# Aedelon/ProteinBERT-PyTorch-Replication

Measured on AMD Instinct MI355X. Metric: sequences/sec (whole node) ProteinBERT pretrain L=512 at 1/2/4/8 MI355X, higher is better.
Workload: dtype bf16; 1 GPU; global_batch=2048, per_gpu_batch=2048, seq_len=512, parallelism=dp1, impl=hip, hip_graph=False

## Files before the change

### proteinbert_pytorch_replication_amd/ops/csrc/wgrad.hip

```cpp
#include "mfma.h"
#include <stdlib.h>

using namespace pbx;
typedef unsigned short bf16_t;

namespace {
constexpr int CH = 128;

constexpr int BM = 128;
constexpr int KS = 9;

__device__ __attribute__((aligned(16))) unsigned int g_zero16[4];
__device__ __attribute__((aligned(16))) unsigned int g_ones16[4] = {~0u, ~0u, ~0u, ~0u};

__device__ __forceinline__ void glds16(const void* src, unsigned char* lds_base) {
  const unsigned dst = __builtin_amdgcn_readfirstlane(
      (unsigned)(size_t)(__attribute__((address_space(3))) unsigned char*)lds_base);
  unsigned keep;
  asm volatile("s_mov_b32 %0, m0\n\ts_mov_b32 m0, %2\n\ts_nop 0\n\tglobal_load_lds_dwordx4 %1, off\n\ts_mov_b32 m0, %0"
               : "=&s"(keep)
               : "v"(src), "s"(dst)
               : "memory");
}

template <int NTAP, int BIAS, typename StageF>
__device__ __forceinline__ void wgrad_tiles(unsigned char* smem, int buf_bytes, long t0, long t1, StageF& stage,
                                            f32x16_t (&acc0)[5], f32x16_t (&acc1)[5], float& bsum, int halo,
                                            int d, int k0, int cig, int lane) {
  const int h = lane >> 5, q = tr_q(lane), tc = tr_c(lane);
  const int aoff = (8 * h + q) * 64 + tc * 2;
  int xoff[NTAP], xoff4[NTAP];
#pragma unroll
  for (int j = 0; j < NTAP; ++j) {
    const int rb = halo + 8 * h + q + (k0 + j - KS / 2) * d;
    xoff[j] = BM * 128 + swz256e(rb, cig * 32 + tc);
    xoff4[j] = BM * 128 + swz256e(rb + 4, cig * 32 + tc);
  }
  if (t0 < t1) stage(t0, smem);
  for (long tile = t0; tile < t1; ++tile) {
    unsigned char* cur = smem + ((tile - t0) & 1) * buf_bytes;
    unsigned char* nxt = smem + (((tile - t0) & 1) ^ 1) * buf_bytes;
    asm volatile("s_waitcnt vmcnt(0)" ::: "memory");
    __syncthreads();
    if (tile + 1 < t1) stage(tile + 1, nxt);
    constexpr int NS = (BM / 16) * NTAP;
    bf16x8 fa0[2], fa1[2], fb[3];
    auto read_a = [&](int kk) {
      const unsigned char* c = cur + kk * 16 * 64;
      fa0[kk & 1] = cat_tr(lds_tr(c, aoff), lds_tr(c, aoff + 256));
      fa1[kk & 1] = cat_tr(lds_tr(c, BM * 64 + aoff), lds_tr(c, BM * 64 + aoff + 256));
    };
    auto read_b = [&](int st) {
      const unsigned char* cx = cur + (st / NTAP) * 16 * 256;
      fb[st % 3] = cat_tr(lds_tr(cx, xoff[st % NTAP]), lds_tr(cx, xoff4[st % NTAP]));
    };
    read_a(0);
    read_b(0);
    read_b(1);
#pragma unroll
    for (int st = 0; st < NS; ++st) {
      const int kk = st / NTAP, j = st % NTAP;
      if (st + 2 < NS) {
        if ((st + 2) % NTAP == 0) read_a((st + 2) / NTAP);
        read_b(st + 2);
      }
      __builtin_amdgcn_sched_barrier(0);
      if (BIAS != 0 && j == 0) {
        typedef __attribute__((ext_vector_type(4))) unsigned int u32x4;
        const u32x4 u = __builtin_bit_cast(u32x4, BIAS == 2 ? fa1[kk & 1] : fa0[kk & 1]);
#pragma unroll
        for (int e = 0; e < 4; ++e)
          bsum += __builtin_bit_cast(float, u[e] << 16) + __builtin_bit_cast(float, u[e] & 0xffff0000u);
      }
      acc0[j] = mfma32(fa0[kk & 1], fb[st % 3], acc0[j]);
      acc1[j] = mfma32(fa1[kk & 1], fb[st % 3], acc1[j]);
    }
  }
}

__global__ void __launch_bounds__(512, 1) wgrad2_kernel(const bf16_t* __restrict__ dy0, const bf16_t* __restrict__ dy1,
                                                        const bf16_t* __restrict__ x, float* __restrict__ slab,
                                                        float* __restrict__ bslab, int B, int L, int dil1,
                                                        int nconv, int R, int buf_bytes, int xlo, int xhi) {
  extern __shared__ __attribute__((aligned(16))) unsigned char smem[];
  const int ntypes = nconv * 2;
  int type, chunk;
  if ((R & 7) == 0) {
    const int id = blockIdx.x, j = id >> 3;
    chunk = (j / ntypes) * 8 + (id & 7);
    type = j - (j / ntypes) * ntypes;
  } else {
    chunk = blockIdx.x / ntypes;
    type = blockIdx.x - chunk * ntypes;
  }
  const int cv = type >> 1, half = type & 1;
  const bf16_t* dy = cv ? dy1 : dy0;
  const int d = cv ? dil1 : 1;
  const int halo = (KS / 2) * d;
  const int XR = BM + 2 * halo;
  const int tid = threadIdx.x, lane = tid & 63, w = __builtin_amdgcn_readfirstlane(tid >> 6);
  const int r = lane & 31, h = lane >> 5;
  const int cig = w & 3;
  const int k0 = w < 4 ? 0 : 5;
  const int ntap = w < 4 ? 5 : 4;
  const int T = (L + BM - 1) / BM;
  const long NT = (long)B * T;
  const long t0 = NT * chunk / R, t1 = NT * (chunk + 1) / R;

  auto stage = [&](long tile, unsigned char* buf) {
    const int b = (int)(tile / T), t = (int)(tile - (tile / T) * T);
    const int pos0 = t * BM;
    const size_t sbase = (size_t)b * L * CH;
    const int n = 16 + XR / 4;
    for (int i = w; i < n; i += 8) {
      if (i < 16) {
        const int sub = i >> 3, row = (i & 7) * 16 + (lane >> 2);
        const int pos = pos0 + row;
        const void* src = pos < L ? (const void*)(dy + sbase + (size_t)pos * CH + half * 64 + sub * 32 + (lane & 3) * 8)
                                  : (const void*)g_zero16;
        glds16(src, buf + sub * (BM * 64) + (i & 7) * 1024);
      } else {
        const int j = i - 16, row = j * 4 + (lane >> 4);
        const int chunk16 = (lane & 15) ^ (((row & 3) << 2) | ((row >> 2) & 3));
        const int pos = pos0 - halo + row;
        const void* src = (pos >= -xlo && pos < L + xhi)
                              ? (const void*)(x + ((ptrdiff_t)b * (L + xlo + xhi) + xlo + pos) * CH + chunk16 * 8)
                              : (const void*)g_zero16;
        glds16(src, buf + BM * 128 + j * 1024);
      }
    }
  };

  f32x16_t acc0[5], acc1[5];
#pragma unroll
  for (int j = 0; j < 5; ++j) {
    acc0[j] = zero16();
    acc1[j] = zero16();
  }
  float bsum = 0.f;
  if (w == 0)
    wgrad_tiles<5, 1>(smem, buf_bytes, t0, t1, stage, acc0, acc1, bsum, halo, d, 0, cig, lane);
  else if (w == 1)
    wgrad_tiles<5, 2>(smem, buf_bytes, t0, t1, stage, acc0, acc1, bsum, halo, d, 0, cig, lane);
  else if (w < 4)
    wgrad_tiles<5, 0>(smem, buf_bytes, t0, t1, stage, acc0, acc1, bsum, halo, d, 0, cig, lane);
  else
    wgrad_tiles<4, 0>(smem, buf_bytes, t0, t1, stage, acc0, acc1, bsum, halo, d, 5, cig, lane);
  float* dst = slab + ((size_t)chunk * nconv + cv) * KS * CH * CH + cig * 32 + r;
#pragma unroll
  for (int j = 0; j < 5; ++j) {
    if (j < ntap) {
      const int k = k0 + j;
#pragma unroll
      for (int i = 0; i < 16; ++i) {
        const int co = half * 64 + (i & 3) + 8 * (i >> 2) + 4 * h;
        dst[((size_t)k * CH + co) * CH] = acc0[j][i];
        dst[((size_t)k * CH + co + 32) * CH] = acc1[j][i];
      }
    }
  }
  if (w < 2) {
    bsum += __shfl_xor(bsum, 32, 64);
    if (h == 0) bslab[((size_t)chunk * nconv + cv) * CH + half * 64 + w * 32 + r] = bsum;
  }
}

__global__ void __launch_bounds__(256) wgrad2_reduce_kernel(const float4* __restrict__ slab,
                                                            const float* __restrict__ bslab, float* __restrict__ dw0,
                                                            float* __restrict__ dw1, float* __restrict__ db0,
                                                            float* __restrict__ db1, int R, int nconv) {
  constexpr int per4 = KS * CH * CH / 4;
  const int total4 = nconv * per4;
  const int nblk_w = (total4 + 63) / 64;
  const int tid = threadIdx.x, col = tid & 63, part = tid >> 6;
  if ((int)blockIdx.x >= nblk_w) {
    const int idx = ((int)blockIdx.x - nblk_w) * 256 + tid;
    if (idx < nconv * CH) {
      float s = 0.f;
      for (int rr = 0; rr < R; ++rr) s += bslab[(size_t)rr * nconv * CH + idx];
      float* db = idx >= CH ? db1 : db0;
      if (db != nullptr) db[idx % CH] += s;
    }
    return;
  }
  __shared__ float4 red[4][64];
  const int idx = blockIdx.x * 64 + col;
  const int r0 = R * part / 4, r1 = R * (part + 1) / 4;
  float4 s = make_float4(0.f, 0.f, 0.f, 0.f);
  if (idx < total4) {
    int rr = r0;
    for (; rr + 8 <= r1; rr += 8) {
      float4 v[8];
#pragma unroll
      for (int u = 0; u < 8; ++u) v[u] = slab[(size_t)(rr + u) * total4 + idx];
#pragma unroll
      for (int u = 0; u < 8; ++u) {
        s.x += v[u].x; s.y += v[u].y; s.z += v[u].z; s.w += v[u].w;
      }
    }
    for (; rr < r1; ++rr) {
      const float4 a = slab[(size_t)rr * total4 + idx];
      s.x += a.x; s.y += a.y; s.z += a.z; s.w += a.w;
    }
  }
  red[part][col] = s;
  __syncthreads();
  if (part == 0 && idx < total4) {
#pragma unroll
    for (int p = 1; p < 4; ++p) {
      const float4 a = red[p][col];
      s.x += a.x; s.y += a.y; s.z += a.z; s.w += a.w;
    }
    const int cv = idx >= per4;
    const int rem = idx - cv * per4;
    const int k = rem / (CH * CH / 4), co = (rem / (CH / 4)) % CH, ci = (rem % (CH / 4)) * 4;
    float* dw = (cv ? dw1 : dw0) + ((size_t)co * CH + ci) * KS + k;
    dw[0] += s.x;
    dw[KS] += s.y;
    dw[2 * KS] += s.z;
    dw[3 * KS] += s.w;
  }
}

bool wgrad2_attr_set = false;
}

PBX_EXPORT int pbx_wgrad2x(const void* dy0, const void* dy1, const void* x, float* slab, float* bslab, float* dw0,
                           float* dw1, float* db0, float* db1, int B, int L, int dil1, int nconv, int R, int xlo,
                           int xhi, hipStream_t st) {
  if (nconv < 1 || nconv > 2 || R < 1 || dil1 < 1 || xlo < 0 || xhi < 0) return (int)hipErrorInvalidValue;
  const int halo_max = (KS / 2) * (nconv > 1 ? dil1 : 1);
  const int buf = BM * 128 + (BM + 2 * halo_max) * 256;
  if (2 * buf > 163840) return (int)hipErrorInvalidValue;
  if (!wgrad2_attr_set) {
    (void)hipFuncSetAttribute((const void*)wgrad2_kernel, hipFuncAttributeMaxDynamicSharedMemorySize, 163840);
    wgrad2_attr_set = true;
  }
  hipLaunchKernelGGL(wgrad2_kernel, dim3(nconv * 2 * R), dim3(512), 2 * buf, st, (const bf16_t*)dy0,
                     (const bf16_t*)dy1, (const bf16_t*)x, slab, bslab, B, L, dil1, nconv, R, buf, xlo, xhi);
  const int total4 = nconv * KS * CH * CH / 4;
  const int nblk = (total4 + 63) / 64 + (nconv * CH + 255) / 256;
  hipLaunchKernelGGL(wgrad2_reduce_kernel, dim3(nblk), dim3(256), 0, st, (const float4*)slab,
                     bslab, dw0, dw1, db0, db1, R, nconv);
  return pbx_launch_status();
}

PBX_EXPORT int pbx_wgrad2(const void* dy0, const void* dy1, const void* x, float* slab, float* bslab, float* dw0,
                          float* dw1, float* db0, float* db1, int B, int L, int dil1, int nconv, int R,
                          hipStream_t st) {
  return pbx_wgrad2x(dy0, dy1, x, slab, bslab, dw0, dw1, db0, db1, B, L, dil1, nconv, R, 0, 0, st);
}

namespace {
constexpr int TBM = 128;

__global__ void __launch_bounds__(512, 1) wgrad_tok_kernel(const long long* __restrict__ tok,
                                                           const bf16_t* __restrict__ dy0,
                                                           const bf16_t* __restrict__ dy1, float* __restrict__ slab,
                                                           int B, int L, int dil1, int R, int V, int buf_bytes) {
  extern __shared__ __attribute__((aligned(16))) unsigned char smem[];
  const int tid = threadIdx.x, lane = tid & 63, w = __builtin_amdgcn_readfirstlane(tid >> 6);
  const int r = lane & 31, h = lane >> 5;
  const int q = tr_q(lane), tc = tr_c(lane);
  const int cv = w >> 2, ct = w & 3;
  const int d = cv ? dil1 : 1;
  const int hal0 = KS / 2, hal1 = (KS / 2) * dil1;
  const int rows0 = TBM + 2 * hal0, rows1 = TBM + 2 * hal1;
  const int T = (L + TBM - 1) / TBM;
  const long NT = (long)B * T;
  const long t0 = NT * blockIdx.x / R, t1 = NT * (blockIdx.x + 1) / R;

  auto stage = [&](long tile, unsigned char* buf) {
    const int b = (int)(tile / T), t = (int)(tile - (tile / T) * T);
    const int pos0 = t * TBM;
    const size_t sbase = (size_t)b * L * CH;
    const int n0 = rows0 / 4, n1 = rows1 / 4;
    for (int i = w; i <= n0 + n1; i += 8) {
      if (i == n0 + n1) {
        const int p = pos0 + 2 * lane;
        const void* src = p < L ? (const void*)(tok + (size_t)b * L + p) : (const void*)g_ones16;
        glds16(src, buf + (rows0 + rows1) * 256);
        continue;
      }
      const int c = i >= n0;
      const int j = c ? i - n0 : i;
      const int hal = c ? hal1 : hal0;
      const bf16_t* dy = c ? dy1 : dy0;
      const int row = j * 4 + (lane >> 4);
      const int chunk16 = (lane & 15) ^ (((row & 3) << 2) | ((row >> 2) & 3));
      const int pos = pos0 - hal + row;
      const void* src = (pos >= 0 && pos < L) ? (const void*)(dy + sbase + (size_t)pos * CH + chunk16 * 8)
                                              : (const void*)g_zero16;
      glds16(src, buf + (c ? rows0 * 256 : 0) + j * 1024);
    }
  };

  f32x16_t acc[KS];
#pragma unroll
  for (int k = 0; k < KS; ++k) acc[k] = zero16();
  const int hal = cv ? hal1 : hal0;
  const int colb = ct * 32 + tc;
  const int cvb = cv ? rows0 * 256 : 0;
  int boff[KS], boff4[KS];
#pragma unroll
  for (int k = 0; k < KS; ++k) {
    const int rb = hal + (KS / 2 - k) * d + 8 * h + q;
    boff[k] = cvb + swz256e(rb, colb);
    boff4[k] = cvb + swz256e(rb + 4, colb);
  }
  const int toff = (rows0 + rows1) * 256 + 8 * h * 8;
  if (t0 < t1) stage(t0, smem);
  for (long tile = t0; tile < t1; ++tile) {
    unsigned char* cur = smem + ((tile - t0) & 1) * buf_bytes;
    unsigned char* nxt = smem + (((tile - t0) & 1) ^ 1) * buf_bytes;
    asm volatile("s_waitcnt vmcnt(0)" ::: "memory");
    __syncthreads();
    if (tile + 1 < t1) stage(tile + 1, nxt);
    constexpr int NS = (TBM / 16) * KS;
    bf16x8 fb[3], fa[2];
    unsigned tk[8];
    auto read_b = [&](int st) {
      const unsigned char* c = cur + (st / KS) * 4096;
      fb[st % 3] = cat_tr(lds_tr(c, boff[st % KS]), lds_tr(c, boff4[st % KS]));
    };
    auto read_tok = [&](int kb) {
      const unsigned* tp = reinterpret_cast<const unsigned*>(cur + toff + kb * 128);
#pragma unroll
      for (int j = 0; j < 8; ++j) tk[j] = tp[2 * j];
    };
    auto make_a = [&](int kb) {
      typedef __attribute__((ext_vector_type(4))) unsigned int u32x4;
      u32x4 o;
#pragma unroll
      for (int e = 0; e < 4; ++e)
        o[e] = (tk[2 * e] == (unsigned)r ? 0x3F80u : 0u) | (tk[2 * e + 1] == (unsigned)r ? 0x3F800000u : 0u);
      fa[kb & 1] = __builtin_bit_cast(bf16x8, o);
    };
    read_tok(0);
    make_a(0);
    read_b(0);
    read_b(1);
#pragma unroll
    for (int st = 0; st < NS; ++st) {
      const int kb = st / KS, k = st % KS;
      if (st + 2 < NS) read_b(st + 2);
      if (k == 3 && kb + 1 < TBM / 16) read_tok(kb + 1);
      if (k == 7 && kb + 1 < TBM / 16) make_a(kb + 1);
      __builtin_amdgcn_sched_barrier(0);
      acc[k] = mfma32(fa[kb & 1], fb[st % 3], acc[k]);
    }
  }
#pragma unroll
  for (int k = 0; k < KS; ++k)
#pragma unroll
    for (int i = 0; i < 16; ++i) {
      const int v = (i & 3) + 8 * (i >> 2) + 4 * h;
      if (v < V) slab[((((size_t)blockIdx.x * 2 + cv) * KS + k) * V + v) * CH + ct * 32 + r] = acc[k][i];
    }
}

__global__ void __launch_bounds__(128) wgrad_tok_finish_kernel(const float* __restrict__ S, const float* __restrict__ E,
                                                               float* __restrict__ dw0, float* __restrict__ dw1,
                                                               float* __restrict__ db0, float* __restrict__ db1,
                                                               int V, const float* __restrict__ W0,
                                                               const float* __restrict__ W1, float* __restrict__ dEslab) {
  __shared__ float sv[KS * 32];
  const int c = blockIdx.x / CH, co = blockIdx.x % CH, ci = threadIdx.x;
  for (int i = threadIdx.x; i < KS * V; i += 128) {
    const int k = i / V, v = i % V;
    sv[k * 32 + v] = S[(((size_t)c * KS + k) * V + v) * CH + co];
  }
  __syncthreads();
  float o[KS];
#pragma unroll
  for (int k = 0; k < KS; ++k) o[k] = 0.f;
  for (int v = 0; v < V; ++v) {
    const float e = bfround(E[v * CH + ci]);
#pragma unroll
    for (int k = 0; k < KS; ++k) o[k] = fmaf(e, sv[k * 32 + v], o[k]);
  }
  float* dw = (c ? dw1 : dw0) + ((size_t)co * CH + ci) * KS;
#pragma unroll
  for (int k = 0; k < KS; ++k) dw[k] += o[k];
  if (ci == 0) {
    float s = 0.f;
    for (int v = 0; v < V; ++v) s += sv[(KS / 2) * 32 + v];
    (c ? db1 : db0)[co] += s;
  }
  if (dEslab != nullptr) {
    const float* wr = (c ? W1 : W0) + ((size_t)co * CH + ci) * KS;
    float wk[KS];
#pragma unroll
    for (int k = 0; k < KS; ++k) wk[k] = bfround(wr[k]);
    for (int v = 0; v < V; ++v) {
      float a = 0.f;
#pragma unroll
      for (int k = 0; k < KS; ++k) a = fmaf(wk[k], sv[k * 32 + v], a);
      dEslab[((size_t)blockIdx.x * V + v) * CH + ci] = a;
    }
  }
}

bool wgrad_tok_attr_set = false;
}

extern "C" int pbx_colsum_add(const float* src, int rows, int cols, float* dst, const float* scale, hipStream_t st);
extern "C" int pbx_colsum_set(const float* src, int rows, int cols, float* dst, const float* scale, hipStream_t st);

PBX_EXPORT int pbx_wgrad_tok_rows(int B, int L) {
  constexpr int cap = 256;
  const long NT = (long)B * ((L + TBM - 1) / TBM);
  return (int)(NT < cap ? NT : cap);
}

PBX_EXPORT int pbx_wgrad_tok(const void* tok, const void* dy0, const void* dy1, const float* E, float* slab, float* S,
                             float* dw0, float* dw1, float* db0, float* db1, int B, int L, int dil1, int V,
                             const float* W0, const float* W1, float* dE, float* dEslab, hipStream_t st) {
  if (V < 1 || V > 32 || dil1 < 1 || (L & 1) || B < 1 || L < 1) return (int)hipErrorInvalidValue;
  if ((dE == nullptr) != (W0 == nullptr) || (dE == nullptr) != (W1 == nullptr) || (dE == nullptr) != (dEslab == nullptr))
    return (int)hipErrorInvalidValue;
  const int buf = (2 * TBM + 8 + 8 * dil1) * 256 + 1024;
  if (2 * buf > 163840) return (int)hipErrorInvalidValue;
  if (!wgrad_tok_attr_set) {
    (void)hipFuncSetAttribute((const void*)wgrad_tok_kernel, hipFuncAttributeMaxDynamicSharedMemorySize, 163840);
    wgrad_tok_attr_set = true;
  }
  const int R = pbx_wgrad_tok_rows(B, L);
  hipLaunchKernelGGL(wgrad_tok_kernel, dim3(R), dim3(512), 2 * buf, st, (const long long*)tok, (const bf16_t*)dy0,
                     (const bf16_t*)dy1, slab, B, L, dil1, R, V, buf);
  const int cols = 2 * KS * V * CH;
  int rc = pbx_colsum_set(slab, R, cols, S, nullptr, st);
  if (rc != 0) return rc;
  hipLaunchKernelGGL(wgrad_tok_finish_kernel, dim3(2 * CH), dim3(128), 0, st, S, E, dw0, dw1, db0, db1, V, W0, W1,
                     dEslab);
  if (dE == nullptr) return pbx_launch_status();
  rc = pbx_launch_status();
  if (rc != 0) return rc;
  return pbx_colsum_add(dEslab, 2 * CH, V * CH, dE, nullptr, st);
}
```

### proteinbert_pytorch_replication_amd/ops/local_track.py

```python
from __future__ import annotations

import ctypes
import os
from typing import List, Dict, Optional, Tuple

import torch

from . import _lib, streams
from ..train.arena import notify_grads_ready
from ..utils.determinism import fused_deterministic
from .global_track import bf16_of

_P, _I, _F, _L = ctypes.c_void_p, ctypes.c_int, ctypes.c_float, ctypes.c_long

_lib.register("pbx_conv_fwd3x", [_P, _P, _P, _P, _P, _P, _P, _P, _P, _P, _I, _I, _I, _I, _I, _I, _P])
_lib.register("pbx_conv_fwd5x", [_P, _P, _P, _P, _P, _P, _P, _P, _P, _P, _I, _I, _I, _I, _I, _I, _P])
_lib.register("pbx_conv_dgrad4x", [_P, _P, _P, _P, _P, _P, _P, _P, _I, _I, _I, _I, _I, _I, _P])
_lib.register("pbx_wgrad2x", [_P, _P, _P, _P, _P, _P, _P, _P, _P, _I, _I, _I, _I, _I, _I, _I, _P])
_lib.register("pbx_pack_conv_frag", [_P, _P, _P, _I, _P])
_lib.register("pbx_wgrad2", [_P, _P, _P, _P, _P, _P, _P, _P, _P, _I, _I, _I, _I, _I, _P])
_lib.register("pbx_wgrad_tok", [_P, _P, _P, _P, _P, _P, _P, _P, _P, _P, _I, _I, _I, _I, _P, _P, _P, _P, _P])
_lib.register("pbx_ln_linear_fwd", [_P, _P, _I, _I, _P, _P, _P, _P, _P, _P, _P, _I, _I, _F, _P])
_lib.register("pbx_pool_fwd", [_P, _P, _P, _P, _P, _P, _P, _I, _I, _I, _F, _P])
_lib.register("pbx_pool_bwd", [_P, _P, _P, _P, _P, _I, _P, _P, _P, _I, _I, _I, _P])
_lib.register("pbx_ln2_linear_bwd", [_P, _P, _P, _P, _I, _P, _P, _P, _P, _I, _I, _P, _P, _P, _P, _P, _P, _P, _P,
                                     _P, _P, _P, _P, _P, _I, _I, _F, _P, _I, _I, _I, _I, _P])
_lib.register("pbx_ln2_bwd_slab_rows", [_I, _I, _I])
_lib.register("pbx_colsum_add", [_P, _I, _I, _P, _P, _P])
_lib.register("pbx_colsum_add2", [_P, _I, _P, _P, _I, _P, _I, _P])
_lib.register("pbx_ln1_finalize", [_P, _P, _P, _I, _I, _P, _I, _P, _P, _P, _I, _I, _F, _I, _P])
_lib.register("pbx_embed_fwd", [_P, _P, _P, _L, _P])
_lib.register("pbx_embed_bwd", [_P, _P, _P, _L, _I, _P, _P])
_lib.register("pbx_conv_fwd3t", [_P, _P, _P, _P, _P, _P, _P, _P, _P, _P, _P, _I, _I, _I, _I, _P])
_lib.register("pbx_conv_dgrad4f", [_P, _P, _P, _I, _I, _P, _I, _P, _P, _P, _P, _P, _P, _P, _P, _P, _I, _I, _I, _I,
                                    _F, _P])
_lib.register("pbx_embed_dpre", [_P, _P, _P, _P, _P, _P, _P, _L, _I, _P, _P])
_lib.register("pbx_embed_bwd_groups", [_L])

CH = 128
PB = 32
LN_EPS = 1e-5


BM1 = 128
def attn_pool_supported(NJ: int) -> bool:
    return NJ in (256, 512)


def conv_tile(L: int) -> int:
    return BM1


def _p(t: Optional[torch.Tensor]):
    return None if t is None else t.data_ptr()


CONV_FWD5 = os.environ.get("PBX_CONV_FWD", "5") == "5"


def conv_dgrad_fin(dh1, s1, st1, T1, BM1, sums1, TS1, g1, gdn, gdw, wtn, wtw, dx, dpn, dpw, dgb, B, L, KS, dil,
                   stream):
    _lib.call("pbx_conv_dgrad4f", dh1.data_ptr(), s1.data_ptr(), st1.data_ptr(), T1, BM1, sums1.data_ptr(),
              TS1, g1.data_ptr(), gdn.data_ptr(), gdw.data_ptr(), wtn.data_ptr(), wtw.data_ptr(),
              dx.data_ptr(), dpn.data_ptr(), dpw.data_ptr(), dgb.data_ptr(), B, L, KS, dil, LN_EPS, stream)


def conv_fwd(x, wpn, wpw, bn, bw, gb, pre_n, pre_w, s1, stats, B, L, KS, dil, stream, xlo: int = 0,
             xhi: int = 0) -> None:
    name = "pbx_conv_fwd5x" if (CONV_FWD5 and KS == 9 and dil == 5) else "pbx_conv_fwd3x"
    _lib.call(name, x.data_ptr(), wpn.data_ptr(), wpw.data_ptr(), bn.data_ptr(), bw.data_ptr(),
              gb.data_ptr(), _p(pre_n), _p(pre_w), s1.data_ptr(), stats.data_ptr(), B, L, KS, dil, xlo, xhi, stream)


def conv_dgrad(ds1, pre_n, pre_w, wtn, wtw, dx, dpn, dpw, B, L, KS, dil, stream, ilo: int = 0, ihi: int = 0) -> None:
    _lib.call("pbx_conv_dgrad4x", ds1.data_ptr(), pre_n.data_ptr(), pre_w.data_ptr(), wtn.data_ptr(),
              wtw.data_ptr(), dx.data_ptr(), dpn.data_ptr(), dpw.data_ptr(), B, L, KS, dil, ilo, ihi, stream)


_DWL_SLAB: Dict[int, torch.Tensor] = {}


def dwl_slab(dev: torch.device) -> Tuple[Optional[int], int]:
    idx = dev.index if dev.index is not None else torch.cuda.current_device()
    s = _DWL_SLAB.get(idx)
    rows = 2 * _num_cus(dev)
    if s is None:
        s = torch.empty(rows * (CH * CH + CH), dtype=torch.float32, device=dev)
        _DWL_SLAB[idx] = s
    return s.data_ptr(), rows


def _num_cus(dev: torch.device) -> int:
    return torch.cuda.get_device_properties(dev).multi_processor_count


def pack_conv(w: torch.Tensor) -> Tuple[torch.Tensor, torch.Tensor]:
    KS = w.shape[2]
    wp = torch.empty((KS, CH, CH), dtype=torch.bfloat16, device=w.device)
    wt = torch.empty_like(wp)
    _lib.call("pbx_pack_conv_frag", w.detach().contiguous().data_ptr(), wp.data_ptr(), wt.data_ptr(), KS,
              _lib.stream_ptr(w.device))
    return wp, wt


def _grad_dst(p: torch.Tensor, shape) -> Tuple[torch.Tensor, bool]:
    g = getattr(p, "grad", None) if getattr(p, "_pbx_arena", False) else None
    if g is not None and g.is_contiguous() and g.dtype == torch.float32 and tuple(g.shape) == tuple(shape):
        return g, True
    return torch.zeros(shape, dtype=torch.float32, device=p.device), False


WGRAD_TAIL_FULL = True
LN2_LATE_FOLD = True
DGRAD_FIN = True
INPUT_BWD_EARLY = True


WGRAD_CU_EIGHTHS = 7


def _wgrad(dy0: torch.Tensor, dy1: Optional[torch.Tensor], x: torch.Tensor, KS: int, dil: int, nconv: int,
           B: int, L: int, outs, full_chip: bool = False, xlo: int = 0, xhi: int = 0):
    dev = x.device
    ntiles = B * ((L + 127) // 128)
    R = max(8, (WGRAD_CU_EIGHTHS * _num_cus(dev) // (16 * nconv)) // 8 * 8)
    if full_chip:
        R = max(8, (_num_cus(dev) // (2 * nconv)) // 8 * 8)
    R = min(R, ntiles)
    slab = torch.empty((R, nconv, KS, CH, CH), dtype=torch.float32, device=dev)
    bslab = torch.empty((R, nconv, CH), dtype=torch.float32, device=dev)
    (dw0, db0) = outs[0]
    (dw1, db1) = outs[1] if nconv > 1 else (None, None)
    if xlo or xhi:
        _lib.call("pbx_wgrad2x", dy0.data_ptr(), _p(dy1), x.data_ptr(), slab.data_ptr(), bslab.data_ptr(),
                  dw0.data_ptr(), _p(dw1), db0.data_ptr(), _p(db1), B, L, dil, nconv, R, xlo, xhi, _lib.stream_ptr(dev))
    else:
        _lib.call("pbx_wgrad2", dy0.data_ptr(), _p(dy1), x.data_ptr(), slab.data_ptr(), bslab.data_ptr(),
                  dw0.data_ptr(), _p(dw1), db0.data_ptr(), _p(db1), B, L, dil, nconv, R, _lib.stream_ptr(dev))
    return [slab, bslab]


WGRAD_TOK = True
EMBED_FOLD = True
EMBED_GATHER = True


def wgrad_tok_ok(tok: Optional[torch.Tensor], emb: Optional[torch.Tensor], L: int, KS: int) -> bool:
    return (WGRAD_TOK and tok is not None and emb is not None and KS == 9 and L % 2 == 0
            and emb.shape[0] <= 32 and emb.shape[1] == CH and tok.dtype == torch.int64 and tok.is_contiguous())


def _wgrad_tok(dy0: torch.Tensor, dy1: torch.Tensor, tok: torch.Tensor, emb: torch.Tensor, dil: int, B: int, L: int,
               outs, demb=None):
    dev = dy0.device
    V = emb.shape[0]
    R = _lib.lib().pbx_wgrad_tok_rows(B, L)
    slab = torch.empty((R, 2, 9, V, CH), dtype=torch.float32, device=dev)
    S = torch.empty((2, 9, V, CH), dtype=torch.float32, device=dev)
    e = emb.detach().float().contiguous()
    (dw0, db0), (dw1, db1) = outs
    w0 = w1 = dE = dEslab = None
    if demb is not None:
        w0, w1 = (w.detach().float().contiguous() for w in demb[:2])
        dE = demb[2]
        dEslab = torch.empty((2 * CH, V, CH), dtype=torch.float32, device=dev)
    _lib.call("pbx_wgrad_tok", tok.data_ptr(), dy0.data_ptr(), dy1.data_ptr(), e.data_ptr(), slab.data_ptr(),
              S.data_ptr(), dw0.data_ptr(), dw1.data_ptr(), db0.data_ptr(), db1.data_ptr(), B, L, dil, V,
              _p(w0), _p(w1), _p(dE), _p(dEslab), _lib.stream_ptr(dev))
    return [slab, S, e, w0, w1, dEslab]


def embed_fold_bwd(tok, emb, ds1, gdn, gdw, dpn, dpw, wn, ww, stream):
    B, L = tok.shape
    dE, direct = _grad_dst(emb, emb.shape)
    slab = None
    if fused_deterministic():
        slab = torch.empty((_lib.lib().pbx_embed_bwd_groups(B * L), emb.shape[0], CH), dtype=torch.float32,
                           device=ds1.device)
    _lib.call("pbx_embed_dpre", tok.data_ptr(), ds1.data_ptr(), gdn.data_ptr(), gdw.data_ptr(), dpn.data_ptr(),
              dpw.data_ptr(), dE.data_ptr(), B * L, emb.shape[0], _p(slab), stream)
    return (wn, ww, dE), direct


class LocalBlockFn(torch.autograd.Function):

    @staticmethod
    def forward(ctx, x, gb, wn, bn, ww, bw, g1, be1, wl, bl, g2, be2, wv_bf16, dil: int, packed=None,
                tail: bool = False, cp=None, tok=None, emb=None, emb_grad: bool = False):
        params = (wn, bn, ww, bw, g1, be1, wl, bl, g2, be2)
        ctx.cp = cp
        if cp is not None:
            g1, be1, g2, be2 = (cp.rows(t) for t in (g1, be1, g2, be2))
        if x is None:
            if not (emb_grad and tok is not None and emb is not None and cp is None):
                raise ValueError("x may be None only for the folded first block (emb_grad with tok / emb)")
            B, L = tok.shape
            xt = torch.empty((B, L, CH), dtype=torch.bfloat16, device=tok.device)
        else:
            B, L, C = x.shape
            assert C == CH and x.dtype == torch.bfloat16 and x.is_contiguous()
            xt = x
        NJ = wv_bf16.shape[0]
        if not attn_pool_supported(NJ):
            raise NotImplementedError(f"HIP attention pool: H * value_dim = {NJ} (kernels built for 256 / 512)")
        KS = wn.shape[2]
        dev = xt.device
        stream = _lib.stream_ptr(dev)
        T1 = (L + BM1 - 1) // BM1
        T2 = (L + PB - 1) // PB
        if packed is not None:
            wpn, wtn, wpw, wtw = packed
        else:
            wpn, wtn = pack_conv(wn)
            wpw, wtw = pack_conv(ww)
        wl_b = bf16_of(wl)
        need_bwd = any(ctx.needs_input_grad)
        pre_n = torch.empty_like(xt) if need_bwd else None
        pre_w = torch.empty_like(xt) if need_bwd else None
        s1 = torch.empty_like(xt)
        st1 = torch.empty((B, T1, 2), dtype=torch.float32, device=dev)
        gb = gb.detach().float().contiguous()
        if x is None:
            x_ext, hlo = None, 0
            emb_b = bf16_of(emb)
            _lib.call("pbx_conv_fwd3t", tok.data_ptr(), emb_b.data_ptr(), wpn.data_ptr(), wpw.data_ptr(),
                      bn.data_ptr(), bw.data_ptr(), gb.data_ptr(), _p(pre_n), _p(pre_w), s1.data_ptr(),
                      st1.data_ptr(), B, L, KS, dil, stream)
        elif cp is None:
            x_ext, hlo = x, 0
            conv_fwd(x, wpn, wpw, bn, bw, gb, pre_n, pre_w, s1, st1, B, L, KS, dil, stream)
        else:
            x_ext, hlo = cp.halo_rows(x), cp.halo
            conv_fwd(x_ext, wpn, wpw, bn, bw, gb, pre_n, pre_w, s1, st1, B, L, KS, dil, stream, hlo, hlo)
            cp.fix_stats(st1, BM1)
        pre_l = torch.empty_like(xt) if need_bwd else None
        s2 = torch.empty_like(xt)
        st2 = torch.empty((B, T2, 2), dtype=torch.float32, device=dev)
        _lib.call("pbx_ln_linear_fwd", s1.data_ptr(), st1.data_ptr(), T1, BM1, g1.data_ptr(), be1.data_ptr(),
                  wl_b.data_ptr(), bl.data_ptr(), _p(pre_l), s2.data_ptr(), st2.data_ptr(), B, L, LN_EPS, stream)
        if cp is not None:
            cp.fix_stats(st2, PB)
        h2 = torch.empty_like(xt)
        TV = (L + 31) // 32
        vpart = torch.empty((B, TV, NJ), dtype=torch.float32, device=dev)
        _lib.call("pbx_pool_fwd", s2.data_ptr(), st2.data_ptr(), g2.data_ptr(), be2.data_ptr(), wv_bf16.data_ptr(),
                  h2.data_ptr(), vpart.data_ptr(), B, L, NJ, LN_EPS, stream)
        ctx.save_for_backward(x_ext, pre_n, pre_w, s1, st1, pre_l, s2, st2, h2, wtn, wtw, wl_b, wv_bf16, g1, be1, g2,
                              be2)
        ctx.hlo = hlo
        ctx.tok = (tok, emb) if cp is None and wgrad_tok_ok(tok, emb, L, KS) else None
        ctx.emb_grad = bool(emb_grad)
        if ctx.emb_grad and (ctx.tok is None or (x is not None and x.requires_grad)):
            raise ValueError("emb_grad needs a token-embedding input without autograd history (wgrad_tok_ok)")
        ctx.meta = (B, L, KS, dil, T1, T2, NJ)
        ctx.tail = bool(tail) and WGRAD_TAIL_FULL
        ctx.set_materialize_grads(False)
        ctx.params = params
        return h2, vpart

    @staticmethod
    def backward(ctx, dh2, dvpart):
        streams.wait_ready(dvpart, dh2)
        (x_ext, pre_n, pre_w, s1, st1, pre_l, s2, st2, h2, wtn, wtw, wl_b, wv_bf16, g1, be1, g2,
         be2) = ctx.saved_tensors
        cp, hlo = ctx.cp, ctx.hlo
        x = s1
        B, L, KS, dil, T1, T2, NJ = ctx.meta
        dev = x.device
        stream = _lib.stream_ptr(dev)
        params = ctx.params
        dsts = [_grad_dst(p, p.shape) for p in params]
        (dwn, _), (dbn, _), (dww, _), (dbw, _), (dg1, _), (dbe1, _), (dwl, _), (dbl, _), (dg2, _), (dbe2, _) = dsts
        if cp is not None:
            dg1, dbe1, dg2, dbe2 = (cp.rows(t) for t in (dg1, dbe1, dg2, dbe2))
        dh2 = None if dh2 is None else dh2.to(torch.bfloat16).contiguous()
        TA = (L + 31) // 32
        if dvpart is None:
            dv, dv_tiles = torch.zeros((B, NJ), dtype=torch.float32, device=dev), 1
        elif dvpart.dim() == 3 and (dvpart.shape[1] == 1 or dvpart.stride(1) == 0):
            dv, dv_tiles = dvpart[:, 0, :].float().contiguous(), 1
        else:
            dv, dv_tiles = dvpart.float().contiguous(), TA
        dh2t = torch.empty_like(x)
        sums2 = torch.empty((B, TA, 2), dtype=torch.float32, device=dev)
        consts = torch.empty((B, 8), dtype=torch.float32, device=dev)
        dgb = torch.empty((B, CH), dtype=torch.float32, device=dev)
        _lib.call("pbx_pool_bwd", h2.data_ptr(), g2.data_ptr(), be2.data_ptr(), _p(dh2), dv.data_ptr(), dv_tiles,
                  wv_bf16.data_ptr(), dh2t.data_ptr(), sums2.data_ptr(), B, L, NJ, stream)
        if cp is not None:
            cp.fix_sums(sums2)
        dh1 = torch.empty_like(x)
        TS1 = (L + 1) // 2
        sums1 = torch.empty((B, TS1, 2), dtype=torch.float32, device=dev)
        det = int(fused_deterministic())
        late_fold = LN2_LATE_FOLD and streams.ENABLED and dev.type == "cuda" and dsts[6][1] and dsts[7][1]
        if late_fold:
            rows = _lib.lib().pbx_ln2_bwd_slab_rows(B, L, det)
            fslab = torch.empty(rows * (CH * CH + CH), dtype=torch.float32, device=dev)
            slab_args = (fslab.data_ptr(), rows)
        else:
            slab_args = dwl_slab(dev)
        _lib.call("pbx_ln2_linear_bwd", dh2t.data_ptr(), s2.data_ptr(), st2.data_ptr(), sums2.data_ptr(), TA,
                  g2.data_ptr(), pre_l.data_ptr(), s1.data_ptr(), st1.data_ptr(), T1, BM1, g1.data_ptr(),
                  be1.data_ptr(), wl_b.data_ptr(), consts.data_ptr(), dh1.data_ptr(), sums1.data_ptr(),
                  dg2.data_ptr(), dbe2.data_ptr(), dg1.data_ptr(), dbe1.data_ptr(), dwl.data_ptr(), dbl.data_ptr(),
                  dgb.data_ptr(), B, L, LN_EPS, *slab_args, det, int(not late_fold), 0, stream)
        if late_fold:
            def fold(slab=fslab, rows=rows, dwl=dwl, dbl=dbl):
                st = _lib.stream_ptr(dev)
                _lib.call("pbx_colsum_add2", slab.data_ptr(), CH * CH, dwl.data_ptr(), slab[rows * CH * CH:].data_ptr(),
                          CH, dbl.data_ptr(), rows, st)
            streams.launch(dev, fold, keep=[fslab], name="wgrad")
        dx = None if ctx.emb_grad else torch.empty_like(x)
        dpn = torch.empty_like(x)
        dpw = torch.empty_like(x)
        if cp is not None:
            cp.fix_sums(sums1)
        fin = (DGRAD_FIN and cp is None and not ctx.emb_grad and KS == 9 and dev.type == "cuda"
               and not fused_deterministic())

        def dgb_ready():
            if ctx.tail and INPUT_BWD_EARLY and streams.ENABLED and dev.type == "cuda":
                streams.fork(dev, "ann")

        if not fin:
            ds1 = torch.empty_like(x)
            _lib.call("pbx_ln1_finalize", dh1.data_ptr(), s1.data_ptr(), st1.data_ptr(), T1, BM1, sums1.data_ptr(),
                      TS1, g1.data_ptr(), ds1.data_ptr(), dgb.data_ptr(), B, L, LN_EPS, int(fused_deterministic()),
                      stream)
            if cp is not None:
                cp.all_reduce_(dgb)
            dgb_ready()
        demb = None
        if fin:
            conv_dgrad_fin(dh1, s1, st1, T1, BM1, sums1, TS1, g1, pre_n, pre_w, wtn, wtw, dx, dpn, dpw, dgb, B, L,
                           KS, dil, stream)
            dgb_ready()
        elif ctx.emb_grad:
            demb, dE_direct = embed_fold_bwd(*ctx.tok, ds1, pre_n, pre_w, dpn, dpw, params[0], params[2], stream)
            dE = demb[2]
        elif cp is None:
            conv_dgrad(ds1, pre_n, pre_w, wtn, wtw, dx, dpn, dpw, B, L, KS, dil, stream)
        else:
            conv_dgrad(*cp.halo_rows_many(ds1, pre_n, pre_w), wtn, wtw, dx, dpn, dpw, B, L,
                       KS, dil, stream, hlo, hlo)
        if ctx.tok is not None:
            tok, emb = ctx.tok
            wg = lambda: _wgrad_tok(dpn, dpw, tok, emb, dil, B, L, [(dwn, dbn), (dww, dbw)], demb)
            keep = [dpn, dpw, tok] + ([demb[2]] if demb is not None else [])
        else:
            wg = lambda: _wgrad(dpn, dpw, x_ext, KS, dil, 2, B, L, [(dwn, dbn), (dww, dbw)],
                                ctx.tail and streams.ENABLED, hlo, hlo)
            keep = [dpn, dpw, x_ext]
        direct = [p for p, (_, d) in zip(params, dsts) if d]
        if demb is not None and dE_direct:
            direct.append(ctx.tok[1])
        if all(dsts[i][1] for i in (0, 1, 2, 3)) and (demb is None or dE_direct) and streams.ENABLED:
            streams.launch(dev, wg, keep=keep, name="wgrad")
        else:
            wg()
        if direct:
            notify_grads_ready(direct)
        pgrads = [None if d else g for (g, d) in dsts]
        gemb = dE if demb is not None and not dE_direct else None
        return (dx, dgb, *pgrads, None, None, None, None, None, None, gemb, None)


def embed_tokens(tokens: torch.Tensor, weight: torch.Tensor) -> torch.Tensor:
    B, L = tokens.shape
    tok = tokens.contiguous()
    out = torch.empty((B, L, weight.shape[1]), dtype=torch.bfloat16, device=tokens.device)
    _lib.call("pbx_embed_fwd", tok.data_ptr(), weight.detach().contiguous().data_ptr(), out.data_ptr(), B * L,
              _lib.stream_ptr(tokens.device))
    return out


class EmbedFn(torch.autograd.Function):

    @staticmethod
    def forward(ctx, tokens, weight):
        B, L = tokens.shape
        V, C = weight.shape
        assert C == CH and V <= 32
        tok = tokens.contiguous()
        out = torch.empty((B, L, C), dtype=torch.bfloat16, device=tokens.device)
        _lib.call("pbx_embed_fwd", tok.data_ptr(), weight.detach().contiguous().data_ptr(), out.data_ptr(), B * L,
                  _lib.stream_ptr(tokens.device))
        ctx.save_for_backward(tok)
        ctx.V = V
        return out

    @staticmethod
    def backward(ctx, dout):
        (tok,) = ctx.saved_tensors
        dE = torch.zeros((ctx.V, CH), dtype=torch.float32, device=tok.device)
        d = dout.to(torch.bfloat16).contiguous()
        slab = None
        if fused_deterministic():
            g = _lib.lib().pbx_embed_bwd_groups(tok.numel())
            slab = torch.empty((g, ctx.V, CH), dtype=torch.float32, device=tok.device)
        _lib.call("pbx_embed_bwd", tok.data_ptr(), d.data_ptr(), dE.data_ptr(), tok.numel(), ctx.V, _lib.ptr(slab),
                  _lib.stream_ptr(tok.device))
        return None, dE


def _wv_bf16(att) -> torch.Tensor:
    Wv = att.Wv
    if isinstance(Wv, torch.nn.Parameter) and Wv.requires_grad:
        return att.value_weight_cat().t().to(torch.bfloat16).contiguous()
    key = (Wv.data_ptr(), Wv._version, Wv.device)
    cached = getattr(att, "_pbx_wv_cache", None)
    if cached is None or cached[0] != key:
        cached = (key, att.value_weight_cat().t().to(torch.bfloat16).contiguous())
        att._pbx_wv_cache = cached
    return cached[1]


def conv_images(wn: torch.Tensor, ww: torch.Tensor):
    KS = wn.shape[2]
    imgs = tuple(torch.empty((KS, CH, CH), dtype=torch.bfloat16, device=wn.device) for _ in range(4))
    return imgs, [(0, wn.detach(), imgs[0], imgs[1], KS, 0), (0, ww.detach(), imgs[2], imgs[3], KS, 0)]


def local_block(x: torch.Tensor, gb: torch.Tensor, blk, packed=None, tail: bool = False,
                cp=None, tok=None, emb=None, emb_grad: bool = False) -> Tuple[torch.Tensor, torch.Tensor]:
    att = blk.global_attention_layer
    wv = _wv_bf16(att)
    nc = blk.local_narrow_conv_layer[0]
    wc = blk.local_wide_conv_layer[0]
    return LocalBlockFn.apply(x, gb, nc.weight, nc.bias, wc.weight, wc.bias, blk.local_norm_1.weight,
                              blk.local_norm_1.bias, blk.local_linear_layer[0].weight, blk.local_linear_layer[0].bias,
                              blk.local_norm_2.weight, blk.local_norm_2.bias, wv, blk.wide_conv_dilation, packed,
                              tail, cp, tok, emb, emb_grad)
```

Before: 103,800 sequences/s.

## Interleave wgrad tile prefetch DMAs into MFMA loop with incremental addressing

Replaces the per-tile staging lambda, which did 64-bit divisions and recomputed addresses, with precomputed stage structs that step base pointers from tile to tile. The global-to-LDS loads for the next tile are now issued one per MFMA step inside the compute loop instead of in a burst before it, so the DMA traffic overlaps the matrix math. This applies to both the conv wgrad and the token wgrad kernels. It also raises the CU fraction given to wgrad chunks from 7/8 to 8/8, which may take compute units away from work running concurrently. The gains depend on the compiler scheduling the issue slots well, and the branchy issue() calls could add instruction overhead.

```diff
diff --git a/proteinbert_pytorch_replication_amd/ops/csrc/wgrad.hip b/proteinbert_pytorch_replication_amd/ops/csrc/wgrad.hip
--- a/proteinbert_pytorch_replication_amd/ops/csrc/wgrad.hip
+++ b/proteinbert_pytorch_replication_amd/ops/csrc/wgrad.hip
@@ -23,8 +23,53 @@
                : "memory");
 }
 
-template <int NTAP, int BIAS, typename StageF>
-__device__ __forceinline__ void wgrad_tiles(unsigned char* smem, int buf_bytes, long t0, long t1, StageF& stage,
+__device__ __forceinline__ unsigned long opaque_addr(const void* p) {
+  unsigned long a = (unsigned long)p;
+  asm volatile("" : "+s"(a));
+  return a;
+}
+
+constexpr int MAXE2 = 10;
+
+struct Stage2 {
+  unsigned long dyb, xb;
+  unsigned long dys, xs;
+  unsigned long zero;
+  int pos0, L;
+  int n, w;
+  int xsh;
+  unsigned xspan;
+  int rowdy, rowx;
+  unsigned dyoff, xoff;
+
+  __device__ __forceinline__ void issue(int e, int nn, unsigned char* buf) const {
+    if (w + 8 * e >= nn) return;
+    if (e < 2) {
+      const unsigned long a = dyb + (unsigned long)(unsigned)pos0 * 256u + dyoff + e * 64;
+      glds16((const void*)(pos0 + rowdy < L ? a : zero), buf + e * (BM * 64) + w * 1024);
+    } else {
+      const int r0 = pos0 + 32 * (e - 2);
+      const unsigned long a = xb + (unsigned long)(unsigned)r0 * 256u + xoff;
+      glds16((const void*)((unsigned)(r0 + rowx + xsh) < xspan ? a : zero),
+             buf + BM * 128 + (w + 8 * (e - 2)) * 1024);
+    }
+  }
+  __device__ __forceinline__ void all(unsigned char* buf) const {
+#pragma unroll
+    for (int e = 0; e < MAXE2; ++e) issue(e, n, buf);
+  }
+  __device__ __forceinline__ void next() {
+    pos0 += BM;
+    if (pos0 >= L) {
+      pos0 = 0;
+      dyb += dys;
+      xb += xs;
+    }
+  }
+};
+
+template <int NTAP, int BIAS>
+__device__ __forceinline__ void wgrad_tiles(unsigned char* smem, int buf_bytes, int nt, Stage2& sg,
                                             f32x16_t (&acc0)[5], f32x16_t (&acc1)[5], float& bsum, int halo,
                                             int d, int k0, int cig, int lane) {
   const int h = lane >> 5, q = tr_q(lane), tc = tr_c(lane);
@@ -36,14 +81,18 @@
     xoff[j] = BM * 128 + swz256e(rb, cig * 32 + tc);
     xoff4[j] = BM * 128 + swz256e(rb + 4, cig * 32 + tc);
   }
-  if (t0 < t1) stage(t0, smem);
-  for (long tile = t0; tile < t1; ++tile) {
-    unsigned char* cur = smem + ((tile - t0) & 1) * buf_bytes;
-    unsigned char* nxt = smem + (((tile - t0) & 1) ^ 1) * buf_bytes;
+  if (nt > 0) {
+    sg.all(smem);
+    sg.next();
+  }
+  for (int it = 0; it < nt; ++it) {
+    unsigned char* cur = smem + (it & 1) * buf_bytes;
+    unsigned char* nxt = smem + ((it & 1) ^ 1) * buf_bytes;
     asm volatile("s_waitcnt vmcnt(0)" ::: "memory");
     __syncthreads();
-    if (tile + 1 < t1) stage(tile + 1, nxt);
+    const int nn = it + 1 < nt ? sg.n : 0;
     constexpr int NS = (BM / 16) * NTAP;
+    static_assert(MAXE2 <= NS, "one DMA per step");
     bf16x8 fa0[2], fa1[2], fb[3];
     auto read_a = [&](int kk) {
       const unsigned char* c = cur + kk * 16 * 64;
@@ -65,6 +114,7 @@
         read_b(st + 2);
       }
       __builtin_amdgcn_sched_barrier(0);
+      if (st < MAXE2) sg.issue(st, nn, nxt);
       if (BIAS != 0 && j == 0) {
         typedef __attribute__((ext_vector_type(4))) unsigned int u32x4;
         const u32x4 u = __builtin_bit_cast(u32x4, BIAS == 2 ? fa1[kk & 1] : fa0[kk & 1]);
@@ -75,6 +125,7 @@
       acc0[j] = mfma32(fa0[kk & 1], fb[st % 3], acc0[j]);
       acc1[j] = mfma32(fa1[kk & 1], fb[st % 3], acc1[j]);
     }
+    sg.next();
   }
 }
 
@@ -106,30 +157,29 @@
   const int T = (L + BM - 1) / BM;
   const long NT = (long)B * T;
   const long t0 = NT * chunk / R, t1 = NT * (chunk + 1) / R;
-
-  auto stage = [&](long tile, unsigned char* buf) {
-    const int b = (int)(tile / T), t = (int)(tile - (tile / T) * T);
-    const int pos0 = t * BM;
-    const size_t sbase = (size_t)b * L * CH;
-    const int n = 16 + XR / 4;
-    for (int i = w; i < n; i += 8) {
-      if (i < 16) {
-        const int sub = i >> 3, row = (i & 7) * 16 + (lane >> 2);
-        const int pos = pos0 + row;
-        const void* src = pos < L ? (const void*)(dy + sbase + (size_t)pos * CH + half * 64 + sub * 32 + (lane & 3) * 8)
-                                  : (const void*)g_zero16;
-        glds16(src, buf + sub * (BM * 64) + (i & 7) * 1024);
-      } else {
-        const int j = i - 16, row = j * 4 + (lane >> 4);
-        const int chunk16 = (lane & 15) ^ (((row & 3) << 2) | ((row >> 2) & 3));
-        const int pos = pos0 - halo + row;
-        const void* src = (pos >= -xlo && pos < L + xhi)
-                              ? (const void*)(x + ((ptrdiff_t)b * (L + xlo + xhi) + xlo + pos) * CH + chunk16 * 8)
-                              : (const void*)g_zero16;
-        glds16(src, buf + BM * 128 + j * 1024);
-      }
-    }
-  };
+  const int nt = (int)(t1 - t0);
+
+  Stage2 sg;
+  {
+    const int b0 = (int)(t0 / T), tt0 = (int)(t0 - (long)b0 * T);
+    const int XS = L + xlo + xhi;
+    sg.dys = (unsigned long)L * CH * 2;
+    sg.xs = (unsigned long)XS * CH * 2;
+    sg.dyb = (unsigned long)dy + (unsigned long)b0 * sg.dys + half * 128;
+    sg.xb = (unsigned long)x + (unsigned long)b0 * sg.xs + (unsigned long)((long)(xlo - halo) * (CH * 2));
+    sg.zero = opaque_addr(g_zero16);
+    sg.pos0 = tt0 * BM;
+    sg.L = L;
+    sg.n = 16 + XR / 4;
+    sg.w = w;
+    sg.xsh = xlo - halo;
+    sg.xspan = (unsigned)XS;
+    sg.rowdy = w * 16 + (lane >> 2);
+    sg.rowx = w * 4 + (lane >> 4);
+    const int chunk16 = (lane & 15) ^ ((((lane >> 4) & 3) << 2) | (w & 3));
+    sg.dyoff = (unsigned)(sg.rowdy * 256 + (lane & 3) * 16);
+    sg.xoff = (unsigned)(sg.rowx * 256 + chunk16 * 16);
+  }
 
   f32x16_t acc0[5], acc1[5];
 #pragma unroll
@@ -139,13 +189,13 @@
   }
   float bsum = 0.f;
   if (w == 0)
-    wgrad_tiles<5, 1>(smem, buf_bytes, t0, t1, stage, acc0, acc1, bsum, halo, d, 0, cig, lane);
+    wgrad_tiles<5, 1>(smem, buf_bytes, nt, sg, acc0, acc1, bsum, halo, d, 0, cig, lane);
   else if (w == 1)
-    wgrad_tiles<5, 2>(smem, buf_bytes, t0, t1, stage, acc0, acc1, bsum, halo, d, 0, cig, lane);
+    wgrad_tiles<5, 2>(smem, buf_bytes, nt, sg, acc0, acc1, bsum, halo, d, 0, cig, lane);
   else if (w < 4)
-    wgrad_tiles<5, 0>(smem, buf_bytes, t0, t1, stage, acc0, acc1, bsum, halo, d, 0, cig, lane);
+    wgrad_tiles<5, 0>(smem, buf_bytes, nt, sg, acc0, acc1, bsum, halo, d, 0, cig, lane);
   else
-    wgrad_tiles<4, 0>(smem, buf_bytes, t0, t1, stage, acc0, acc1, bsum, halo, d, 5, cig, lane);
+    wgrad_tiles<4, 0>(smem, buf_bytes, nt, sg, acc0, acc1, bsum, halo, d, 5, cig, lane);
   float* dst = slab + ((size_t)chunk * nconv + cv) * KS * CH * CH + cig * 32 + r;
 #pragma unroll
   for (int j = 0; j < 5; ++j) {
@@ -253,6 +303,50 @@
 
 namespace {
 constexpr int TBM = 128;
+constexpr int MAXET = 10;
+
+struct StageTok {
+  unsigned long dyb0, dyb1, tokb;
+  unsigned long dys, toks;
+  unsigned long zero, ones;
+  int pos0, L;
+  int n0, n, w;
+  int hal1;
+  int lane, lrow;
+  unsigned lx;
+
+  __device__ __forceinline__ void issue(int e, int nn, unsigned char* buf) const {
+    const int i = w + 8 * e;
+    if (i > nn) return;
+    if (i == n) {
+      const int p = pos0 + 2 * lane;
+      unsigned long a = tokb + (unsigned long)(unsigned)p * 8u;
+      asm volatile("" : "+v"(a));
+      glds16((const void*)(p < L ? a : ones), buf + n * 1024);
+      return;
+    }
+    const bool c = i >= n0;
+    const int j = c ? i - n0 : i;
+    const int r0 = pos0 - (c ? hal1 : KS / 2) + 4 * j;
+    const unsigned lo = (unsigned)(lrow * 256) + ((lx ^ (unsigned)(j & 3)) << 4);
+    unsigned long a = (c ? dyb1 : dyb0) + (unsigned long)((long)r0 * 256) + lo;
+    asm volatile("" : "+v"(a));
+    glds16((const void*)((unsigned)(r0 + lrow) < (unsigned)L ? a : zero), buf + i * 1024);
+  }
+  __device__ __forceinline__ void all(unsigned char* buf) const {
+#pragma unroll
+    for (int e = 0; e < MAXET; ++e) issue(e, n, buf);
+  }
+  __device__ __forceinline__ void next() {
+    pos0 += TBM;
+    if (pos0 >= L) {
+      pos0 = 0;
+      dyb0 += dys;
+      dyb1 += dys;
+      tokb += toks;
+    }
+  }
+};
 
 __global__ void __launch_bounds__(512, 1) wgrad_tok_kernel(const long long* __restrict__ tok,
                                                            const bf16_t* __restrict__ dy0,
@@ -270,30 +364,28 @@
   const long NT = (long)B * T;
   const long t0 = NT * blockIdx.x / R, t1 = NT * (blockIdx.x + 1) / R;
 
-  auto stage = [&](long tile, unsigned char* buf) {
-    const int b = (int)(tile / T), t = (int)(tile - (tile / T) * T);
-    const int pos0 = t * TBM;
-    const size_t sbase = (size_t)b * L * CH;
-    const int n0 = rows0 / 4, n1 = rows1 / 4;
-    for (int i = w; i <= n0 + n1; i += 8) {
-      if (i == n0 + n1) {
-        const int p = pos0 + 2 * lane;
-        const void* src = p < L ? (const void*)(tok + (size_t)b * L + p) : (const void*)g_ones16;
-        glds16(src, buf + (rows0 + rows1) * 256);
-        continue;
-      }
-      const int c = i >= n0;
-      const int j = c ? i - n0 : i;
-      const int hal = c ? hal1 : hal0;
-      const bf16_t* dy = c ? dy1 : dy0;
-      const int row = j * 4 + (lane >> 4);
-      const int chunk16 = (lane & 15) ^ (((row & 3) << 2) | ((row >> 2) & 3));
-      const int pos = pos0 - hal + row;
-      const void* src = (pos >= 0 && pos < L) ? (const void*)(dy + sbase + (size_t)pos * CH + chunk16 * 8)
-                                              : (const void*)g_zero16;
-      glds16(src, buf + (c ? rows0 * 256 : 0) + j * 1024);
-    }
-  };
+  const int nt = (int)(t1 - t0);
+
+  StageTok sg;
+  {
+    const int b0 = (int)(t0 / T), tt0 = (int)(t0 - (long)b0 * T);
+    sg.dys = (unsigned long)L * CH * 2;
+    sg.toks = (unsigned long)L * 8;
+    sg.dyb0 = (unsigned long)dy0 + (unsigned long)b0 * sg.dys;
+    sg.dyb1 = (unsigned long)dy1 + (unsigned long)b0 * sg.dys;
+    sg.tokb = (unsigned long)tok + (unsigned long)b0 * sg.toks;
+    sg.zero = opaque_addr(g_zero16);
+    sg.ones = opaque_addr(g_ones16);
+    sg.pos0 = tt0 * TBM;
+    sg.L = L;
+    sg.n0 = rows0 / 4;
+    sg.n = rows0 / 4 + rows1 / 4;
+    sg.w = w;
+    sg.hal1 = hal1;
+    sg.lane = lane;
+    sg.lrow = lane >> 4;
+    sg.lx = (unsigned)((lane & 15) ^ (((lane >> 4) & 3) << 2));
+  }
 
   f32x16_t acc[KS];
 #pragma unroll
@@ -309,14 +401,18 @@
     boff4[k] = cvb + swz256e(rb + 4, colb);
   }
   const int toff = (rows0 + rows1) * 256 + 8 * h * 8;
-  if (t0 < t1) stage(t0, smem);
-  for (long tile = t0; tile < t1; ++tile) {
-    unsigned char* cur = smem + ((tile - t0) & 1) * buf_bytes;
-    unsigned char* nxt = smem + (((tile - t0) & 1) ^ 1) * buf_bytes;
+  if (nt > 0) {
+    sg.all(smem);
+    sg.next();
+  }
+  for (int it = 0; it < nt; ++it) {
+    unsigned char* cur = smem + (it & 1) * buf_bytes;
+    unsigned char* nxt = smem + ((it & 1) ^ 1) * buf_bytes;
     asm volatile("s_waitcnt vmcnt(0)" ::: "memory");
     __syncthreads();
-    if (tile + 1 < t1) stage(tile + 1, nxt);
+    const int nn = it + 1 < nt ? sg.n : -1;
     constexpr int NS = (TBM / 16) * KS;
+    static_assert(MAXET <= NS, "one DMA per step");
     bf16x8 fb[3], fa[2];
     unsigned tk[8];
     auto read_b = [&](int st) {
@@ -347,8 +443,10 @@
       if (k == 3 && kb + 1 < TBM / 16) read_tok(kb + 1);
       if (k == 7 && kb + 1 < TBM / 16) make_a(kb + 1);
       __builtin_amdgcn_sched_barrier(0);
+      if (st < MAXET) sg.issue(st, nn, nxt);
       acc[k] = mfma32(fa[kb & 1], fb[st % 3], acc[k]);
     }
+    sg.next();
   }
 #pragma unroll
   for (int k = 0; k < KS; ++k)
diff --git a/proteinbert_pytorch_replication_amd/ops/local_track.py b/proteinbert_pytorch_replication_amd/ops/local_track.py
--- a/proteinbert_pytorch_replication_amd/ops/local_track.py
+++ b/proteinbert_pytorch_replication_amd/ops/local_track.py
@@ -116,7 +116,7 @@
 INPUT_BWD_EARLY = True
 
 
-WGRAD_CU_EIGHTHS = 7
+WGRAD_CU_EIGHTHS = 8
 
 
 def _wgrad(dy0: torch.Tensor, dy1: Optional[torch.Tensor], x: torch.Tensor, KS: int, dil: int, nconv: int,
```

After: 106,100 sequences/s, median of 6. 2.2% higher.
